# lesliegaga/GPT-SoVITS

Hardware: AMD Instinct MI355X
Metric: synthesised audio sec/sec (1/RTF), v2 pipeline (higher is better)
Workload: dtype f16

## Files before the change

gpt-sovits_amd/csrc/conv_launch.h:

```cpp
#pragma once
#include <stdlib.h>

#include <algorithm>
#include <type_traits>

#include "common.h"

namespace gsv {

int launch_gemm_sk(int dtype, const ConvArgs& a, hipStream_t s);
int launch_conv_wide(int dtype, const ConvArgs& a, hipStream_t s);
int launch_gemm_lds(int dtype, const ConvArgs& a, hipStream_t s);
int launch_conv_narrow(int dtype, const ConvArgs& a, hipStream_t s);
int launch_conv_lds(int dtype, const ConvArgs& a, hipStream_t s);

inline const char* env_switch(const char* name) { return getenv(name); }
inline long long env_number(const char* name, long long unset) { const char* v = env_switch(name); return v ? atoll(v) : unset; }
inline char env_first(const char* name) { const char* v = env_switch(name); return v ? v[0] : '\0'; }
struct ConvSwitches {
  bool no_conv_lds = env_switch("GSV_NO_CONV_LDS");
  bool trace_conv_gemm = env_switch("GSV_TRACE_CONV_GEMM");
  long long gemm_small_tiles = env_number("GSV_CONV_GEMM_SMALL_TILES", 64);
  bool no_gemm_sk = env_switch("GSV_NO_GEMM_SK");
  int sk_max_tiles = (int)env_number("GSV_SK_MAX_TILES", 160);
  bool gemm_t64 = env_first("GSV_GEMM_T64") != '0';
  int t64_slab = (int)env_number("GSV_T64_SLAB", 128);
  bool no_conv_wide = env_switch("GSV_NO_CONV_WIDE");
  int wide_waves = (int)env_number("GSV_WIDE_WAVES", 8);
  bool wide_prof = env_switch("GSV_WIDE_PROF");
  int gemm_xcd = env_first("GSV_GEMM_XCD") == '0' ? 0 : env_first("GSV_GEMM_XCD") == '1' ? 1 : 2;
  int gemm_waves = (int)env_number("GSV_GEMM_WAVES", 8);
  long long gemm_w8_max_tiles = env_number("GSV_GEMM_W8_MAX_TILES", 256);
  bool no_persist = env_switch("GSV_CONV_NO_PERSIST");
  bool no_persist64 = env_switch("GSV_CONV_NO_PERSIST64");
  int narrow_per_cu = std::max(1, (int)env_number("GSV_NARROW_PER_CU", 3));
  bool narrow_prof = env_switch("GSV_NARROW_PROF");
  bool no_half_tile = env_switch("GSV_CONV_NO_HALF_TILE");
  bool half_always = env_switch("GSV_CONV_HALF_ALWAYS");
  int half_waves = (int)env_number("GSV_CONV_HALF_WAVES", 8);
  int tile_waves = (int)env_number("GSV_CONV_TILE_WAVES", 8);
  bool no_conv_pair = env_switch("GSV_NO_CONV_PAIR");
  bool no_conv_pair64 = env_switch("GSV_NO_CONV_PAIR64");
  int pair_per_cu = std::max(1, (int)env_number("GSV_PAIR_PER_CU", 3));
};
inline const ConvSwitches& conv_switches() {
  static const ConvSwitches sw{};
  return sw;
}

template <auto Kern, int LdsCap, typename... Args>
int launch_routed(unsigned long long route, dim3 grid, dim3 block, size_t lds, hipStream_t s, Args... args) {
  if constexpr (LdsCap > 0) {
    static bool cap_set = false;
    if (!cap_set) {
      GSV_HIP(hipFuncSetAttribute((const void*)Kern, hipFuncAttributeMaxDynamicSharedMemorySize, LdsCap));
      cap_set = true;
    }
  }
  set_conv_route(route);
  GSV_LAUNCH(Kern, grid, block, lds, s, args...);
  return GSV_OK;
}
constexpr int LDS_CAP = 160 * 1024;

template <typename F> int with_flags(F&& f) { return f(); }
template <typename F, typename... Bools> int with_flags(F&& f, bool b, Bools... rest) {
  return with_flags([&](auto... tail) { return b ? f(std::true_type{}, tail...) : f(std::false_type{}, tail...); }, rest...);
}

template <int G> bool operands_aligned(const ConvArgs& a) {
  return a.ldx % G == 0 && a.ldw % G == 0 && (uintptr_t)a.x % 16 == 0 && (uintptr_t)a.w % 16 == 0;
}

struct TileStamps {
  unsigned long long* dev = nullptr;
  int calls = 0;
  unsigned long long* buffer(bool on) {
    if (on && !dev) { (void)hipMalloc((void**)&dev, 64 * 8); (void)hipMemset(dev, 0, 64 * 8); }
    return dev;
  }
  void report(hipStream_t s, int max_stamps, const char* fmt, ...) {
    if (!dev || ++calls != 3) return;
    (void)hipStreamSynchronize(s);
    unsigned long long hp[64];
    (void)hipMemcpy(hp, dev, sizeof(hp), hipMemcpyDeviceToHost);
    va_list ap;
    va_start(ap, fmt);
    vfprintf(stderr, fmt, ap);
    va_end(ap);
    for (int i = 1; i < max_stamps && hp[i]; ++i) fprintf(stderr, " %.2f", (double)(hp[i] - hp[0]) / 100.0);
    fprintf(stderr, "\n");
  }
};

}
```

gpt-sovits_amd/csrc/conv_wide.hip:

```cpp
#include "conv_launch.h"

namespace gsv {

namespace {

typedef _Float16 T;
typedef h8 F;
typedef _Float16 T4 __attribute__((ext_vector_type(4)));

__device__ __forceinline__ void mma32w(f16v& acc, const h8& a, const h8& b) { acc = __builtin_amdgcn_mfma_f32_32x32x16_f16(a, b, acc, 0, 0, 0); }
__device__ __forceinline__ h8 lrelu8w(h8 v, float s) { h8 t = v * (_Float16)s; return __builtin_elementwise_max(v, t); }
__device__ __forceinline__ h8 relu8w(h8 v) { return __builtin_elementwise_max(v, (h8){0, 0, 0, 0, 0, 0, 0, 0}); }

template <bool RES, bool ACCU, int NW>
__global__ __launch_bounds__(NW * 64) void conv_wide_f16_kernel(ConvArgs a, int rows_win, int ntiles) {
  constexpr int G = 8, KC = 16, CC = 128, CT = 128, TM = 2, TN = NW == 8 ? 2 : 4, WN = NW == 8 ? 4 : 2, NT = NW * 64;
  constexpr int LDX = CC + G, VPR = CC / G;
  constexpr int WLOADS = CT * VPR / NT;
  constexpr int XB = (306 * VPR + NT - 1) / NT;
  constexpr int LDO = CT + 4, PR = TN * 32, IPR = CT / 4, NI = PR * IPR / NT;
  extern __shared__ __attribute__((aligned(16))) unsigned char smem[];
  T* xs = (T*)smem;
  T* ws = xs + (size_t)306 * LDX;
  float* os = (float*)smem;
  static_assert((size_t)PR * LDO * 4 <= (size_t)306 * LDX * 2, "epilogue tile must fit in the window");
  const int tid = threadIdx.x, lane = tid & 63, wave = tid >> 6;
  const int r = lane & 31, h = lane >> 5;
  const int wm = wave / WN, wn = wave % WN;
  const T* __restrict__ x = (const T*)a.x;
  const T* __restrict__ w = (const T*)a.w;
  const int total = rows_win * VPR;
  const int ecg = tid % IPR, ec = 4 * ecg;
  f4 ebias = (f4){0.f, 0.f, 0.f, 0.f};
  if (a.bias) for (int j = 0; j < 4; ++j) ebias[j] = a.bias[ec + j];

  auto load_w = [&](int tap, F* regs) {
#pragma unroll
    for (int i = 0; i < WLOADS; ++i) {
      const int v = tid + i * NT;
      const int row = v / VPR, col = v - row * VPR;
      regs[i] = *(const F*)(w + (long long)row * a.ldw + (long long)tap * CC + col * G);
    }
  };
  auto store_w = [&](int buf, const F* regs) {
#pragma unroll
    for (int i = 0; i < WLOADS; ++i) {
      const int v = tid + i * NT;
      const int row = v / VPR, col = v - row * VPR;
      *(F*)(ws + ((size_t)buf * CT + row) * LDX + col * G) = regs[i];
    }
  };
  auto load_window = [&](int tile, F* regs) {
    const int win_start = tile * 256 - a.pad;
#pragma unroll
    for (int i = 0; i < XB; ++i) {
      const int v = min(tid + i * NT, total - 1);
      const int row = v / VPR, col = v - row * VPR;
      const int ti = win_start + row;
      const F val = *(const F*)(x + (long long)min(max(ti, 0), a.T_in - 1) * a.ldx + col * G);
      regs[i] = (ti >= 0 && ti < a.T_in) ? val : (F){0, 0, 0, 0, 0, 0, 0, 0};
    }
  };
  auto store_window = [&](const F* regs) {
#pragma unroll
    for (int i = 0; i < XB; ++i) {
      const int v = tid + i * NT;
      if (v < total) {
        const int row = v / VPR, col = v - row * VPR;
        F val = regs[i];
        if (a.pre_act == ACT_LRELU) val = lrelu8w(val, a.pre_slope);
        else if (a.pre_act == ACT_RELU) val = relu8w(val);
        *(F*)(xs + (size_t)row * LDX + col * G) = val;
      }
    }
  };
  int tile = blockIdx.x;
  {
    F first[XB], w0[WLOADS];
    load_window(min(tile, ntiles - 1), first);
    load_w(0, w0);
    store_window(first);
    store_w(0, w0);
  }
  lds_barrier();
  for (; tile < ntiles; tile += gridDim.x) {
    const int t0 = tile * 256;
    const bool pf = a.prof && blockIdx.x == 100 && tile == 100 + 3 * (int)gridDim.x && tid == 0;
    int pi = 0;
#define WSTAMP() do { if (pf) a.prof[pi++] = __builtin_amdgcn_s_memrealtime(); } while (0)
    WSTAMP();
    F nxt[XB];
    load_window(min(tile + (int)gridDim.x, ntiles - 1), nxt);
    T4 rv[RES ? NI : 1];
    auto load_res_pass = [&](int pass) {
#pragma unroll
      for (int e = 0; e < (RES ? NI : 0); ++e) {
        const int t = min(t0 + pass * PR + (tid + e * NT) / IPR, a.T_out - 1);
        rv[e] = *(const T4*)((const T*)a.res + (long long)t * a.ldr + ec);
      }
    };
    if (RES) load_res_pass(0);
    f16v acc[TM][TN];
#pragma unroll
    for (int m = 0; m < TM; ++m)
#pragma unroll
      for (int n = 0; n < TN; ++n)
#pragma unroll
        for (int i = 0; i < 16; ++i) acc[m][n][i] = 0.f;
    for (int tap = 0; tap < a.taps; ++tap) {
      const int buf = tap & 1;
      F wnx[WLOADS];
      const bool more = tap + 1 < a.taps;
      if (more) load_w(tap + 1, wnx);
      const int shift = tap * a.dil;
      const T* wb = ws + (size_t)buf * CT * LDX;
#pragma unroll 2
      for (int ks = 0; ks < CC / KC; ++ks) {
        const int kk = ks * KC + G * h;
        F af[TM], bf[TN];
#pragma unroll
        for (int m = 0; m < TM; ++m) af[m] = *(const F*)(wb + (size_t)((wm * TM + m) * 32 + r) * LDX + kk);
#pragma unroll
        for (int n = 0; n < TN; ++n) bf[n] = *(const F*)(xs + (size_t)((wn * TN + n) * 32 + r + shift) * LDX + kk);
#pragma unroll
        for (int m = 0; m < TM; ++m)
#pragma unroll
          for (int n = 0; n < TN; ++n) mma32w(acc[m][n], af[m], bf[n]);
      }
      if (more) {
        store_w(buf ^ 1, wnx);
        lds_barrier();
      }
      WSTAMP();
    }
#pragma unroll
    for (int pass = 0; pass < WN; ++pass) {
      lds_barrier();
      WSTAMP();
      if (wn == pass) {
#pragma unroll
        for (int m = 0; m < TM; ++m)
#pragma unroll
          for (int n = 0; n < TN; ++n) {
            const int tl = n * 32 + r;
#pragma unroll
            for (int g = 0; g < 4; ++g) {
              const int cl = (wm * TM + m) * 32 + 8 * g + 4 * h;
              *(f4*)(os + (size_t)tl * LDO + cl) = (f4){acc[m][n][4 * g], acc[m][n][4 * g + 1], acc[m][n][4 * g + 2], acc[m][n][4 * g + 3]};
            }
          }
      }
      WSTAMP();
      lds_barrier();
      WSTAMP();
      T4 ya[ACCU ? NI : 1];
#pragma unroll
      for (int e = 0; e < (ACCU ? NI : 0); ++e) {
        const int t = min(t0 + pass * PR + (tid + e * NT) / IPR, a.T_out - 1);
        ya[e] = *(const T4*)((const T*)a.y + (long long)t * a.ldy + ec);
      }
      auto items = [&](auto act_tag) {
#pragma unroll
        for (int e = 0; e < NI; ++e) {
          const int tl = (tid + e * NT) / IPR;
          const int t = t0 + pass * PR + tl;
          if (t >= a.T_out) continue;
          const f4 av = *(const f4*)(os + (size_t)tl * LDO + 4 * ecg);
          float v[4];
#pragma unroll
          for (int j = 0; j < 4; ++j) {
            float u = av[j] + ebias[j];
            if (RES) u += (float)rv[e][j];
            u *= a.scale;
            u = post_act_c<decltype(act_tag)::value>(a.post_act, u);
            if (ACCU) u += (float)ya[e][j];
            v[j] = u;
          }
          *(T4*)((T*)a.y + (long long)t * a.ldy + ec) = (T4){(T)v[0], (T)v[1], (T)v[2], (T)v[3]};
        }
      };
      GSV_ACT_DISPATCH(a.post_act, items);
      if (RES && pass + 1 < WN) load_res_pass(pass + 1);
      WSTAMP();
    }
    F w0[WLOADS];
    load_w(0, w0);
    lds_barrier();
    store_window(nxt);
    store_w(0, w0);
    lds_barrier();
    WSTAMP();
  }
}

}

int launch_conv_wide(int dtype, const ConvArgs& a, hipStream_t s) {
  const ConvSwitches& sw = conv_switches();
  if (sw.no_conv_wide || dtype != GSV_F16) return 1;
  if (a.Cin != 128 || a.Cout != 128 || a.Z != 1 || a.stride != 1 || a.ups_u > 0 || a.dil < 1 || a.gate || a.taps < 2) return 1;
  if (a.out_f32 || a.res_f32 || a.y_col0 != 0 || a.T_virt < 16384 || a.T_out != a.T_virt || a.T_in < 1) return 1;
  if (!operands_aligned<8>(a) || a.ldy % 4 != 0 || (a.res && a.ldr % 4 != 0)) return 1;
  const int span = (a.taps - 1) * a.dil;
  if (span > 50 || a.pad < 0 || a.pad > span) return 1;
  const int rows_win = 256 + span;
  const int ntiles = cdiv(a.T_virt, 256);
  const size_t lds = ((size_t)306 + 2 * 128) * 136 * 2;
  const int grid = std::min(ntiles, 256);
  static TileStamps stamps;
  ConvArgs b = a;
  b.prof = stamps.buffer(sw.wide_prof);
  GSV_RC(with_flags([&](auto R, auto A, auto W8) {
    constexpr int NW = W8.value ? 8 : 4;
    return launch_routed<conv_wide_f16_kernel<R.value, A.value, NW>, LDS_CAP>(
        route_code(ROUTE_CONV_WIDE, GSV_F16, NW, 0, 0, 0, 0, route_flags(R.value, A.value)), dim3(grid), dim3(NW * 64), lds, s, b, rows_win, ntiles);
  }, a.res != nullptr, a.accumulate != 0, sw.wide_waves == 8));
  stamps.report(s, 24, "[wide prof] taps %d:", a.taps);
  return GSV_OK;
}

}
```

Before: 2786.

## Give each wave a private weight slab in the wide conv kernel

```diff
diff --git a/gpt-sovits_amd/csrc/conv_launch.h b/gpt-sovits_amd/csrc/conv_launch.h
--- a/gpt-sovits_amd/csrc/conv_launch.h
+++ b/gpt-sovits_amd/csrc/conv_launch.h
@@ -26,7 +26,7 @@
   bool gemm_t64 = env_first("GSV_GEMM_T64") != '0';
   int t64_slab = (int)env_number("GSV_T64_SLAB", 128);
   bool no_conv_wide = env_switch("GSV_NO_CONV_WIDE");
-  int wide_waves = (int)env_number("GSV_WIDE_WAVES", 8);
+  bool wide_staged = env_switch("GSV_WIDE_STAGED");
   bool wide_prof = env_switch("GSV_WIDE_PROF");
   int gemm_xcd = env_first("GSV_GEMM_XCD") == '0' ? 0 : env_first("GSV_GEMM_XCD") == '1' ? 1 : 2;
   int gemm_waves = (int)env_number("GSV_GEMM_WAVES", 8);
diff --git a/gpt-sovits_amd/csrc/conv_wide.hip b/gpt-sovits_amd/csrc/conv_wide.hip
--- a/gpt-sovits_amd/csrc/conv_wide.hip
+++ b/gpt-sovits_amd/csrc/conv_wide.hip
@@ -12,9 +12,198 @@
 __device__ __forceinline__ h8 lrelu8w(h8 v, float s) { h8 t = v * (_Float16)s; return __builtin_elementwise_max(v, t); }
 __device__ __forceinline__ h8 relu8w(h8 v) { return __builtin_elementwise_max(v, (h8){0, 0, 0, 0, 0, 0, 0, 0}); }
 
-template <bool RES, bool ACCU, int NW>
-__global__ __launch_bounds__(NW * 64) void conv_wide_f16_kernel(ConvArgs a, int rows_win, int ntiles) {
-  constexpr int G = 8, KC = 16, CC = 128, CT = 128, TM = 2, TN = NW == 8 ? 2 : 4, WN = NW == 8 ? 4 : 2, NT = NW * 64;
+template <bool RES, bool ACCU>
+__global__ __launch_bounds__(512) void conv_wide_f16_kernel(ConvArgs a, int rows_win, int ntiles) {
+  constexpr int G = 8, KC = 16, CC = 128, CT = 128, KS = CC / KC, TN = 4, NT = 512;
+  constexpr int LDX = CC + G, VPR = CC / G;
+  constexpr int XB = (306 * VPR + NT - 1) / NT;
+  constexpr int LDO = CT + 4, PR = TN * 32, IPR = CT / 4, NI = PR * IPR / NT;
+  extern __shared__ __attribute__((aligned(16))) unsigned char smem[];
+  T* xs = (T*)smem;
+  T* ps = xs + (size_t)306 * LDX;
+  float* os = (float*)ps;
+  static_assert((size_t)PR * LDO * 4 <= (size_t)8 * 32 * LDX * 2, "epilogue tile must fit in the weight images");
+  const int tid = threadIdx.x, lane = tid & 63, wave = tid >> 6;
+  const int r = lane & 31, h = lane >> 5;
+  const int wm = wave >> 1, wn = wave & 1;
+  const T* __restrict__ x = (const T*)a.x;
+  auto w_base = [&](int l) { return (const T*)a.w + (long long)(wm * 32 + (l >> 3)) * a.ldw + (l & 7) * G; };
+  T* pw = ps + (size_t)wave * 32 * LDX;
+  T* pdst = pw + (size_t)(lane >> 3) * LDX + (lane & 7) * G;
+  const T* pa = pw + (size_t)r * LDX + G * h;
+  const int ec = 4 * (tid % IPR);
+  f4 ebias = (f4){0.f, 0.f, 0.f, 0.f};
+  if (a.bias) for (int j = 0; j < 4; ++j) ebias[j] = a.bias[ec + j];
+
+  auto load_window = [&](int tile, F* regs, int row0, int wcol) {
+    const int win_start = tile * 256 - a.pad;
+#pragma unroll
+    for (int i = 0; i < XB; ++i) {
+      const int ti = win_start + min(row0 + i * (NT / VPR), rows_win - 1);
+      const F val = *(const F*)(x + (long long)min(max(ti, 0), a.T_in - 1) * a.ldx + wcol);
+      regs[i] = (ti >= 0 && ti < a.T_in) ? val : (F){0, 0, 0, 0, 0, 0, 0, 0};
+    }
+  };
+  auto store_window = [&](const F* regs, int row0, int wcol) {
+#pragma unroll
+    for (int i = 0; i < XB; ++i) {
+      const int row = row0 + i * (NT / VPR);
+      if (row < rows_win) {
+        F val = regs[i];
+        if (a.pre_act == ACT_LRELU) val = lrelu8w(val, a.pre_slope);
+        else if (a.pre_act == ACT_RELU) val = relu8w(val);
+        *(F*)(xs + (size_t)row * LDX + wcol) = val;
+      }
+    }
+  };
+  int tile = blockIdx.x;
+  F stg[KS];
+  auto w_load = [&](const T* wsrc, int tap, int c) {
+#pragma unroll
+    for (int jj = 0; jj < 4; ++jj) stg[4 * c + jj] = *(const F*)(wsrc + (long long)(jj * 8) * a.ldw + tap * CC + c * 64);
+  };
+  auto w_store = [&](int c) {
+#pragma unroll
+    for (int jj = 0; jj < 4; ++jj) *(F*)(pdst + (size_t)(jj * 8) * LDX + c * 64) = stg[4 * c + jj];
+  };
+  {
+    F first[XB];
+    load_window(min(tile, ntiles - 1), first, tid / VPR, (tid % VPR) * G);
+    w_load(w_base(lane), 0, 0);
+    w_load(w_base(lane), 0, 1);
+    store_window(first, tid / VPR, (tid % VPR) * G);
+  }
+  lds_barrier();
+  for (; tile < ntiles; tile += gridDim.x) {
+    const int t0 = tile * 256;
+    const bool pf = a.prof && blockIdx.x == 100 && tile == 100 + 3 * (int)gridDim.x && tid == 0;
+    int pi = 0;
+#define WSTAMP() do { if (pf) a.prof[pi++] = __builtin_amdgcn_s_memrealtime(); } while (0)
+    WSTAMP();
+    int lt = tid;
+    asm volatile("" : "+v"(lt));
+    const int row0 = lt / VPR, wcol = (lt % VPR) * G, er0 = lt / IPR, lc = 4 * (lt % IPR);
+    const T* wsrc = w_base(lt & 63);
+    w_store(0);
+    w_store(1);
+    asm volatile("" ::: "memory");
+    w_load(wsrc, 1, 0);
+    w_load(wsrc, 1, 1);
+    T4 rv[2][RES ? NI : 1], ya[2][ACCU ? NI : 1];
+    auto load_res = [&](int pass) {
+#pragma unroll
+      for (int e = 0; e < (RES ? NI : 0); ++e) {
+        const int t = min(t0 + pass * PR + er0 + e * (NT / IPR), a.T_out - 1);
+        rv[pass][e] = *(const T4*)((const T*)a.res + (long long)t * a.ldr + lc);
+      }
+    };
+    auto load_acc = [&](int pass) {
+#pragma unroll
+      for (int e = 0; e < (ACCU ? NI : 0); ++e) {
+        const int t = min(t0 + pass * PR + er0 + e * (NT / IPR), a.T_out - 1);
+        ya[pass][e] = *(const T4*)((const T*)a.y + (long long)t * a.ldy + lc);
+      }
+    };
+    f16v acc[TN];
+#pragma unroll
+    for (int n = 0; n < TN; ++n)
+#pragma unroll
+      for (int i = 0; i < 16; ++i) acc[n][i] = 0.f;
+    auto tap_mma = [&](int tap, auto last_tag) {
+      const int tap2 = min(tap + 2, a.taps - 1);
+      const T* xb = xs + (size_t)(wn * PR + r + tap * a.dil) * LDX + G * h;
+      F bf[2][TN];
+#pragma unroll
+      for (int n = 0; n < TN; ++n) bf[0][n] = *(const F*)(xb + (size_t)n * 32 * LDX);
+#pragma unroll
+      for (int c = 0; c < 2; ++c) {
+#pragma unroll
+        for (int ks = 4 * c; ks < 4 * c + 4; ++ks) {
+          const F af = *(const F*)(pa + ks * KC);
+          if (ks + 1 < KS) {
+#pragma unroll
+            for (int n = 0; n < TN; ++n) bf[(ks + 1) & 1][n] = *(const F*)(xb + (size_t)n * 32 * LDX + (ks + 1) * KC);
+          }
+#pragma unroll
+          for (int n = 0; n < TN; ++n) mma32w(acc[n], af, bf[ks & 1][n]);
+          __builtin_amdgcn_sched_barrier(0);
+        }
+        if (!decltype(last_tag)::value) {
+          asm volatile("" ::: "memory");
+          w_store(c);
+          asm volatile("" ::: "memory");
+          w_load(wsrc, tap2, c);
+          __builtin_amdgcn_sched_barrier(0);
+        }
+      }
+      WSTAMP();
+    };
+    tap_mma(0, std::false_type{});
+    for (int tap = 1; tap + 1 < a.taps; ++tap) tap_mma(tap, std::false_type{});
+    load_res(0);
+    load_acc(0);
+    tap_mma(a.taps - 1, std::true_type{});
+    load_res(1);
+    load_acc(1);
+    F nxt[XB];
+    load_window(min(tile + (int)gridDim.x, ntiles - 1), nxt, row0, wcol);
+    lds_barrier();
+    WSTAMP();
+#pragma unroll
+    for (int pass = 0; pass < 2; ++pass) {
+      if (pass == 1) {
+        lds_barrier();
+        WSTAMP();
+      }
+      if (wn == pass) {
+#pragma unroll
+        for (int n = 0; n < TN; ++n) {
+          const int tl = n * 32 + r;
+#pragma unroll
+          for (int g = 0; g < 4; ++g) {
+            const int cl = wm * 32 + 8 * g + 4 * h;
+            *(f4*)(os + (size_t)tl * LDO + cl) = (f4){acc[n][4 * g], acc[n][4 * g + 1], acc[n][4 * g + 2], acc[n][4 * g + 3]};
+          }
+        }
+      }
+      lds_barrier();
+      WSTAMP();
+      auto items = [&](auto act_tag) {
+#pragma unroll
+        for (int e = 0; e < NI; ++e) {
+          const int tl = er0 + e * (NT / IPR);
+          const int t = t0 + pass * PR + tl;
+          if (t >= a.T_out) continue;
+          const f4 av = *(const f4*)(os + (size_t)tl * LDO + lc);
+          float v[4];
+#pragma unroll
+          for (int j = 0; j < 4; ++j) {
+            float u = av[j] + ebias[j];
+            if (RES) u += (float)rv[pass][e][j];
+            u *= a.scale;
+            u = post_act_c<decltype(act_tag)::value>(a.post_act, u);
+            if (ACCU) u += (float)ya[pass][e][j];
+            v[j] = u;
+          }
+          *(T4*)((T*)a.y + (long long)t * a.ldy + lc) = (T4){(T)v[0], (T)v[1], (T)v[2], (T)v[3]};
+        }
+      };
+      GSV_ACT_DISPATCH(a.post_act, items);
+    }
+    store_window(nxt, row0, wcol);
+    int le = lane;
+    asm volatile("" : "+v"(le));
+    w_load(w_base(le), 0, 0);
+    w_load(w_base(le), 0, 1);
+    lds_barrier();
+    WSTAMP();
+#undef WSTAMP
+  }
+}
+
+template <bool RES, bool ACCU>
+__global__ __launch_bounds__(512) void conv_wide_staged_f16_kernel(ConvArgs a, int rows_win, int ntiles) {
+  constexpr int G = 8, KC = 16, CC = 128, CT = 128, TM = 2, TN = 2, WN = 4, NT = 512;
   constexpr int LDX = CC + G, VPR = CC / G;
   constexpr int WLOADS = CT * VPR / NT;
   constexpr int XB = (306 * VPR + NT - 1) / NT;
@@ -190,6 +379,7 @@
     store_w(0, w0);
     lds_barrier();
     WSTAMP();
+#undef WSTAMP
   }
 }
 
@@ -210,11 +400,13 @@
   static TileStamps stamps;
   ConvArgs b = a;
   b.prof = stamps.buffer(sw.wide_prof);
-  GSV_RC(with_flags([&](auto R, auto A, auto W8) {
-    constexpr int NW = W8.value ? 8 : 4;
-    return launch_routed<conv_wide_f16_kernel<R.value, A.value, NW>, LDS_CAP>(
-        route_code(ROUTE_CONV_WIDE, GSV_F16, NW, 0, 0, 0, 0, route_flags(R.value, A.value)), dim3(grid), dim3(NW * 64), lds, s, b, rows_win, ntiles);
-  }, a.res != nullptr, a.accumulate != 0, sw.wide_waves == 8));
+  GSV_RC(with_flags([&](auto R, auto A, auto S) {
+    const unsigned long long route = route_code(ROUTE_CONV_WIDE, GSV_F16, 8, 0, 0, 0, 0, route_flags(R.value, A.value));
+    if constexpr (S.value)
+      return launch_routed<conv_wide_staged_f16_kernel<R.value, A.value>, LDS_CAP>(route, dim3(grid), dim3(512), lds, s, b, rows_win, ntiles);
+    else
+      return launch_routed<conv_wide_f16_kernel<R.value, A.value>, LDS_CAP>(route, dim3(grid), dim3(512), lds, s, b, rows_win, ntiles);
+  }, a.res != nullptr, a.accumulate != 0, sw.wide_staged));
   stamps.report(s, 24, "[wide prof] taps %d:", a.taps);
   return GSV_OK;
 }
```

Result: no change. 2800 (median of 3 runs) (+0.5%).
